# williamleif/GraphSAGE

Measured on NVIDIA H100. Metric: seed_nodes_per_sec, higher is better.
Workload: dtype f32

## Files before the change

### graphsage_b200/csrc/gemm_tc.cu

```cuda
#include "tc_common.cuh"

namespace gs {

constexpr int TC_THREADS = 256;

struct TcPart {
  const float* A;
  int64_t lda;
  int32_t K;
  int32_t N;
  int32_t kblocks;
  int32_t ntiles;
  int64_t img_off;
  const float* B;
  int64_t ldb;
};

struct TcParams {
  TcPart p[2];
  int32_t n_parts;
  int32_t combine;
  int64_t M;
  const float* bias;
  int32_t act;
  float* out;
  int64_t ldo;
  int32_t tiles_n0;
  gs_gemm_row_ids rid[2];
};

template <int MODE>
__global__ void __launch_bounds__(256) pack_b_kernel(TcParams prm, unsigned char* __restrict__ ws) {
  constexpr int BK = MODE == 2 ? 64 : 32;
  constexpr int EPC = MODE == 2 ? 8 : 4;
  constexpr int NIMG = MODE == 0 ? 2 : 1;
  int unit = blockIdx.x;
  int pi = 0;
  if (prm.n_parts == 2 && unit >= prm.p[0].ntiles * prm.p[0].kblocks) {
    unit -= prm.p[0].ntiles * prm.p[0].kblocks;
    pi = 1;
  }
  const TcPart& P = prm.p[pi];
  const int nt = unit / P.kblocks, kb = unit % P.kblocks;
  unsigned char* img = ws + P.img_off + ((int64_t)(nt * P.kblocks + kb) * NIMG) * TC_TILE_BYTES;
  for (int q = threadIdx.x; q < 128 * 8; q += blockDim.x) {
    const int c = q >> 7, n = q & 127;
    const int gn = nt * TC_BN + n;
    const int k0 = kb * BK + c * EPC;
    float w[EPC];
#pragma unroll
    for (int e = 0; e < EPC; ++e) w[e] = (gn < P.N && k0 + e < P.K) ? P.B[(int64_t)(k0 + e) * P.ldb + gn] : 0.f;
    const uint32_t off = sw128_off(n, c);
    if constexpr (MODE == 2) {
      __nv_bfloat162 h[4];
#pragma unroll
      for (int e = 0; e < 4; ++e) h[e] = __floats2bfloat162_rn(w[2 * e], w[2 * e + 1]);
      *reinterpret_cast<uint4*>(img + off) = *reinterpret_cast<uint4*>(h);
    } else {
      uint4 hi;
      hi.x = tf32_mask(w[0]); hi.y = tf32_mask(w[1]); hi.z = tf32_mask(w[2]); hi.w = tf32_mask(w[3]);
      *reinterpret_cast<uint4*>(img + off) = hi;
      if constexpr (MODE == 0) {
        uint4 lo;
        lo.x = tf32_mask(w[0] - __uint_as_float(hi.x)); lo.y = tf32_mask(w[1] - __uint_as_float(hi.y));
        lo.z = tf32_mask(w[2] - __uint_as_float(hi.z)); lo.w = tf32_mask(w[3] - __uint_as_float(hi.w));
        *reinterpret_cast<uint4*>(img + TC_TILE_BYTES + off) = lo;
      }
    }
  }
}

template <int MODE>
struct TcCfg {
  static constexpr int BK = MODE == 2 ? 64 : 32;
  static constexpr int NIMG = MODE == 0 ? 2 : 1;
  static constexpr int IMG_BYTES = NIMG * TC_TILE_BYTES;
  static constexpr int STAGES = MODE == 0 ? 3 : 4;
  static constexpr int STAGE_BYTES = 2 * IMG_BYTES;
  static constexpr int SMEM_BYTES = STAGES * STAGE_BYTES + 1024;
  static constexpr int CPT = 4;
};

template <int MODE>
__device__ __forceinline__ void load_a_chunk(const TcPart& P, int64_t arow, int gcol, bool vec, float (&v)[8]) {
  constexpr int EPC = MODE == 2 ? 8 : 4;
#pragma unroll
  for (int e = 0; e < 8; ++e) v[e] = 0.f;
  if (arow < 0) return;
  const float* src = P.A + arow * P.lda + gcol;
  if (vec && gcol + EPC <= P.K) {
    float4 a = ldg_nc_f4(reinterpret_cast<const float4*>(src));
    v[0] = a.x; v[1] = a.y; v[2] = a.z; v[3] = a.w;
    if constexpr (EPC == 8) {
      float4 b = ldg_nc_f4(reinterpret_cast<const float4*>(src) + 1);
      v[4] = b.x; v[5] = b.y; v[6] = b.z; v[7] = b.w;
    }
  } else {
#pragma unroll
    for (int e = 0; e < EPC; ++e)
      if (gcol + e < P.K) v[e] = __ldg(src + e);
  }
}

template <int MODE>
__device__ __forceinline__ void store_a_chunk(unsigned char* tile, int row, int c, const float (&v)[8]) {
  const uint32_t off = sw128_off(row, c);
  if constexpr (MODE == 2) {
    __nv_bfloat162 h[4];
#pragma unroll
    for (int e = 0; e < 4; ++e) h[e] = __floats2bfloat162_rn(v[2 * e], v[2 * e + 1]);
    *reinterpret_cast<uint4*>(tile + off) = *reinterpret_cast<uint4*>(h);
  } else {
    uint4 hi;
    hi.x = tf32_mask(v[0]); hi.y = tf32_mask(v[1]); hi.z = tf32_mask(v[2]); hi.w = tf32_mask(v[3]);
    *reinterpret_cast<uint4*>(tile + off) = hi;
    if constexpr (MODE == 0) {
      uint4 lo;
      lo.x = tf32_mask(v[0] - __uint_as_float(hi.x)); lo.y = tf32_mask(v[1] - __uint_as_float(hi.y));
      lo.z = tf32_mask(v[2] - __uint_as_float(hi.z)); lo.w = tf32_mask(v[3] - __uint_as_float(hi.w));
      *reinterpret_cast<uint4*>(tile + TC_TILE_BYTES + off) = lo;
    }
  }
}

template <int MODE>
__global__ void __launch_bounds__(TC_THREADS, 1) sage_gemm_tc_kernel(const __grid_constant__ TcParams prm,
                                                                     const unsigned char* __restrict__ ws) {
  using C = TcCfg<MODE>;
  extern __shared__ unsigned char smem_raw[];
  __shared__ __align__(8) uint64_t full[C::STAGES];

  unsigned char* smem = reinterpret_cast<unsigned char*>((reinterpret_cast<uintptr_t>(smem_raw) + 1023) & ~(uintptr_t)1023);
  const int tid = threadIdx.x, wg = tid >> 7, lane = tid & 31, wq = (tid >> 5) & 3;

  const int64_t m0 = (int64_t)blockIdx.x * TC_BM;
  int part_lo = 0, part_hi = prm.n_parts, ntile = blockIdx.y, col_off = 0;
  if (prm.combine == GS_COMBINE_CONCAT && prm.n_parts == 2) {
    if ((int)blockIdx.y < prm.tiles_n0) part_hi = 1;
    else { part_lo = 1; ntile = blockIdx.y - prm.tiles_n0; col_off = prm.p[0].N; }
  }
  const int N = prm.p[part_lo].N;
  int total_it = 0;
  for (int pi = part_lo; pi < part_hi; ++pi) total_it += prm.p[pi].kblocks;
  auto locate = [&](int it, int& pi, int& kb) {
    pi = part_lo; kb = it;
    while (kb >= prm.p[pi].kblocks) { kb -= prm.p[pi].kblocks; ++pi; }
  };

  if (tid == 0) {
    for (int s = 0; s < C::STAGES; ++s) mbar_init(&full[s], 1);
    fence_mbar_init();
  }
  __syncthreads();

  auto post = [&](int it) {
    if (tid != 0 || it >= total_it) return;
    int pi, kb;
    locate(it, pi, kb);
    const TcPart& P = prm.p[pi];
    const int s = it % C::STAGES;
    unsigned char* st = smem + (size_t)s * C::STAGE_BYTES;
    mbar_expect_tx(&full[s], C::IMG_BYTES);
    bulk_g2s(st + C::IMG_BYTES, ws + P.img_off + ((int64_t)ntile * P.kblocks + kb) * C::IMG_BYTES, C::IMG_BYTES, &full[s]);
  };
  int64_t arow_lo[C::CPT], arow_hi[C::CPT];
#pragma unroll
  for (int i = 0; i < C::CPT; ++i) {
    const int64_t r = m0 + ((tid + TC_THREADS * i) >> 3);
    arow_lo[i] = gemm_a_row(prm.rid[part_lo], prm.M, r);
    arow_hi[i] = part_hi - part_lo == 2 ? gemm_a_row(prm.rid[part_lo + 1], prm.M, r) : -1;
  }
  float cur[C::CPT][8];
  auto fetch = [&](int it) {
    int pi, kb;
    locate(it, pi, kb);
    const TcPart& P = prm.p[pi];
    const bool vec = ((P.lda & 3) == 0) && ((reinterpret_cast<uintptr_t>(P.A) & 15u) == 0);
#pragma unroll
    for (int i = 0; i < C::CPT; ++i) {
      const int q = tid + TC_THREADS * i;
      load_a_chunk<MODE>(P, pi == part_lo ? arow_lo[i] : arow_hi[i], kb * C::BK + (q & 7) * (MODE == 2 ? 8 : 4), vec, cur[i]);
    }
  };

  for (int j = 0; j < C::STAGES - 1; ++j) post(j);
  fetch(0);

  float acc[64];
#pragma unroll
  for (int i = 0; i < 64; ++i) acc[i] = 0.f;
  for (int it = 0; it < total_it; ++it) {
    const int s = it % C::STAGES;
    unsigned char* st = smem + (size_t)s * C::STAGE_BYTES;
#pragma unroll
    for (int i = 0; i < C::CPT; ++i) {
      const int q = tid + TC_THREADS * i;
      store_a_chunk<MODE>(st, q >> 3, q & 7, cur[i]);
    }
    fence_proxy_async();
    __syncthreads();
    post(it + C::STAGES - 1);
    if (it + 1 < total_it) fetch(it + 1);
    mbar_wait(&full[s], (uint32_t)(it / C::STAGES) & 1u);
    const uint32_t a_base = smem_u32(st) + (uint32_t)(wg * 64 * 128), b_base = smem_u32(st + C::IMG_BYTES);
    const uint64_t a_hi = make_smem_desc(a_base), b_hi = make_smem_desc(b_base);
    const uint64_t a_lo = make_smem_desc(a_base + TC_TILE_BYTES), b_lo = make_smem_desc(b_base + TC_TILE_BYTES);
    acc_fence(acc);
    wgmma_fence();
#pragma unroll
    for (int k = 0; k < 4; ++k) {
      const uint64_t koff = (uint64_t)((k * 32) >> 4);
      wgmma_m64n128<MODE == 2>(acc, a_hi + koff, b_hi + koff, (it > 0 || k > 0) ? 1u : 0u);
      if constexpr (MODE == 0) {
        wgmma_m64n128<false>(acc, a_hi + koff, b_lo + koff, 1u);
        wgmma_m64n128<false>(acc, a_lo + koff, b_hi + koff, 1u);
      }
    }
    wgmma_commit();
    wgmma_wait<0>();
    acc_fence(acc);
  }

#pragma unroll
  for (int h = 0; h < 2; ++h) {
    const int64_t grow = m0 + wg * 64 + wq * 16 + (lane >> 2) + 8 * h;
    if (grow >= prm.M) continue;
    float* dst_row = prm.out + grow * prm.ldo + col_off;
#pragma unroll
    for (int j = 0; j < 16; ++j) {
      const int gn = ntile * TC_BN + 8 * j + 2 * (lane & 3);
      float v[2];
#pragma unroll
      for (int e = 0; e < 2; ++e) {
        v[e] = acc[4 * j + 2 * h + e];
        if (prm.bias && gn + e < N) v[e] += prm.bias[col_off + gn + e];
        if (prm.act == GS_ACT_RELU) v[e] = fmaxf(v[e], 0.f);
      }
      float* dst = dst_row + gn;
      if (gn + 2 <= N && (reinterpret_cast<uintptr_t>(dst) & 7u) == 0) {
        *reinterpret_cast<float2*>(dst) = make_float2(v[0], v[1]);
      } else {
        if (gn < N) dst[0] = v[0];
        if (gn + 1 < N) dst[1] = v[1];
      }
    }
  }
}

static int mode_of(int32_t math) { return math == GS_MATH_TF32X3 ? 0 : math == GS_MATH_TF32 ? 1 : 2; }

static void fill_parts(TcParams& prm, int64_t M, const gs_gemm_part* parts, int32_t n_parts, int mode) {
  const int BK = mode == 2 ? 64 : 32;
  const int nimg = mode == 0 ? 2 : 1;
  memset(&prm, 0, sizeof(prm));
  prm.n_parts = n_parts;
  prm.M = M;
  int64_t off = 0;
  for (int i = 0; i < n_parts; ++i) {
    TcPart& P = prm.p[i];
    P.A = parts[i].A; P.lda = parts[i].lda; P.K = parts[i].K; P.N = parts[i].N;
    P.B = parts[i].B; P.ldb = parts[i].ldb;
    P.kblocks = (P.K + BK - 1) / BK;
    P.ntiles = (P.N + TC_BN - 1) / TC_BN;
    P.img_off = off;
    off += (int64_t)P.kblocks * P.ntiles * nimg * TC_TILE_BYTES;
  }
  prm.tiles_n0 = prm.p[0].ntiles;
}

int64_t sage_gemm_tc_workspace(int64_t M, const gs_gemm_part* parts, int32_t n_parts, int32_t math) {
  TcParams prm;
  fill_parts(prm, M, parts, n_parts, mode_of(math));
  const TcPart& L = prm.p[n_parts - 1];
  const int nimg = mode_of(math) == 0 ? 2 : 1;
  return L.img_off + (int64_t)L.kblocks * L.ntiles * nimg * TC_TILE_BYTES;
}

template <int MODE>
static int32_t launch_pack(const TcParams& prm, unsigned char* ws, cudaStream_t st) {
  int units = prm.p[0].ntiles * prm.p[0].kblocks + (prm.n_parts == 2 ? prm.p[1].ntiles * prm.p[1].kblocks : 0);
  pack_b_kernel<MODE><<<units, 256, 0, st>>>(prm, ws);
  return launch_check("pack_b_kernel");
}

template <int MODE>
static int32_t launch_tc(const TcParams& prm, const unsigned char* ws, cudaStream_t st) {
  using C = TcCfg<MODE>;
  const int32_t rc_attr = ensure_dyn_smem((const void*)sage_gemm_tc_kernel<MODE>, C::SMEM_BYTES);
  if (rc_attr != GS_OK) return rc_attr;
  int tiles_n = prm.p[0].ntiles;
  if (prm.combine == GS_COMBINE_CONCAT && prm.n_parts == 2) tiles_n += prm.p[1].ntiles;
  dim3 grid((unsigned)((prm.M + TC_BM - 1) / TC_BM), (unsigned)tiles_n);
  sage_gemm_tc_kernel<MODE><<<grid, TC_THREADS, C::SMEM_BYTES, st>>>(prm, ws);
  return launch_check("sage_gemm_tc_kernel");
}

int32_t sage_gemm_tc_pack(const gs_gemm_part* parts, int32_t n_parts, int32_t math, void* workspace, cudaStream_t st) {
  GS_REQUIRE(workspace != nullptr && (reinterpret_cast<uintptr_t>(workspace) & 127u) == 0,
             "gs_sage_gemm_pack: workspace must be non-NULL and 128-byte aligned");
  const int mode = mode_of(math);
  TcParams prm;
  fill_parts(prm, 0, parts, n_parts, mode);
  unsigned char* ws = (unsigned char*)workspace;
  if (mode == 0) return launch_pack<0>(prm, ws, st);
  if (mode == 1) return launch_pack<1>(prm, ws, st);
  return launch_pack<2>(prm, ws, st);
}

int32_t sage_gemm_tc(int64_t M, const gs_gemm_part* parts, const gs_gemm_row_ids* row_ids, int32_t n_parts, int32_t combine,
                     const float* bias, int32_t act, int32_t math, float* out, int64_t ldo, const void* workspace,
                     cudaStream_t st) {
  GS_REQUIRE(workspace != nullptr, "gs_sage_gemm: tensor-core math modes need the workspace (gs_sage_gemm_workspace_bytes)");
  GS_REQUIRE((reinterpret_cast<uintptr_t>(workspace) & 127u) == 0, "gs_sage_gemm: workspace must be 128-byte aligned");
  const int mode = mode_of(math);
  TcParams prm;
  fill_parts(prm, M, parts, n_parts, mode);
  for (int i = 0; row_ids && i < n_parts; ++i) prm.rid[i] = row_ids[i];
  prm.combine = combine;
  prm.bias = bias;
  prm.act = act;
  prm.out = out;
  prm.ldo = ldo;
  const unsigned char* ws = (const unsigned char*)workspace;
  if (mode == 0) return launch_tc<0>(prm, ws, st);
  if (mode == 1) return launch_tc<1>(prm, ws, st);
  return launch_tc<2>(prm, ws, st);
}

}
```

### graphsage_b200/csrc/layer_small.cu

```cuda
#include "common.cuh"

namespace gs {

constexpr int LS_ROWS = 4;
constexpr int LS_THREADS = 512;

struct LsParams {
  const float* src;
  int64_t n_src_rows, pitch;
  int32_t F;
  gs_segment seg;
  int32_t include_self;
  gs_gemm_part p[2];
  int32_t n_parts, combine;
  const float* bias;
  int32_t act, l2norm;
  float* out;
  int64_t ldo;
  uint64_t* counter_dev;
  uint64_t counter_inc;
  int32_t vec;
};

__device__ __forceinline__ int64_t ls_clamp(int64_t id, int64_t n) { return (id < 0 || id >= n) ? n - 1 : id; }

__global__ void __launch_bounds__(LS_THREADS) sage_layer_small_kernel(const __grid_constant__ LsParams prm) {
  extern __shared__ float sm[];
  const int F = prm.F;
  float* xs = sm;
  float* xm = sm + LS_ROWS * F;
  const gs_segment& sg = prm.seg;
  const int k = sg.k;
  const int64_t row0 = (int64_t)blockIdx.x * LS_ROWS;
  if (prm.vec) {
    const int f4 = F >> 2;
    for (int p = threadIdx.x; p < f4 * LS_ROWS; p += LS_THREADS) {
      const int r = p / f4, c4 = p - r * f4;
      const int64_t i = row0 + r;
      float4 acc = make_float4(0.f, 0.f, 0.f, 0.f), sv = acc;
      if (i < sg.n) {
        const int64_t srow = ls_clamp(sg.self_ids ? (int64_t)sg.self_ids[i] : sg.self_row0 + i, prm.n_src_rows);
        sv = ldg_nc_f4(reinterpret_cast<const float4*>(prm.src + srow * prm.pitch) + c4);
        for (int j0 = 0; j0 < k; j0 += 5) {
          float4 v[5];
#pragma unroll
          for (int u = 0; u < 5; ++u) {
            v[u] = make_float4(0.f, 0.f, 0.f, 0.f);
            if (j0 + u < k) {
              const int64_t nr = ls_clamp(sg.neigh_ids ? (int64_t)sg.neigh_ids[i * k + j0 + u] : sg.neigh_row0 + i * k + j0 + u,
                                          prm.n_src_rows);
              v[u] = ldg_nc_f4(reinterpret_cast<const float4*>(prm.src + nr * prm.pitch) + c4);
            }
          }
#pragma unroll
          for (int u = 0; u < 5; ++u) { acc.x += v[u].x; acc.y += v[u].y; acc.z += v[u].z; acc.w += v[u].w; }
        }
        const float div = (float)(k + (prm.include_self ? 1 : 0));
        if (prm.include_self) { acc.x += sv.x; acc.y += sv.y; acc.z += sv.z; acc.w += sv.w; }
        acc.x /= div; acc.y /= div; acc.z /= div; acc.w /= div;
      }
      reinterpret_cast<float4*>(xs + r * F)[c4] = sv;
      reinterpret_cast<float4*>(xm + r * F)[c4] = acc;
    }
  } else
  for (int c = threadIdx.x; c < F; c += LS_THREADS) {
    float acc[LS_ROWS], sv[LS_ROWS];
#pragma unroll
    for (int r = 0; r < LS_ROWS; ++r) {
      acc[r] = 0.f;
      const int64_t i = row0 + r;
      sv[r] = 0.f;
      if (i < sg.n) {
        const int64_t srow = ls_clamp(sg.self_ids ? (int64_t)sg.self_ids[i] : sg.self_row0 + i, prm.n_src_rows);
        sv[r] = prm.src[srow * prm.pitch + c];
      }
    }
    for (int j0 = 0; j0 < k; j0 += 5) {
      float v[LS_ROWS][5];
#pragma unroll
      for (int r = 0; r < LS_ROWS; ++r) {
        const int64_t i = row0 + r;
#pragma unroll
        for (int u = 0; u < 5; ++u) {
          v[r][u] = 0.f;
          if (i < sg.n && j0 + u < k) {
            const int64_t nr = ls_clamp(sg.neigh_ids ? (int64_t)sg.neigh_ids[i * k + j0 + u] : sg.neigh_row0 + i * k + j0 + u,
                                        prm.n_src_rows);
            v[r][u] = prm.src[nr * prm.pitch + c];
          }
        }
      }
#pragma unroll
      for (int r = 0; r < LS_ROWS; ++r)
#pragma unroll
        for (int u = 0; u < 5; ++u) acc[r] += v[r][u];
    }
#pragma unroll
    for (int r = 0; r < LS_ROWS; ++r) {
      float a = acc[r];
      if (prm.include_self) a += sv[r];
      a /= (float)(k + (prm.include_self ? 1 : 0));
      xs[r * F + c] = sv[r];
      xm[r * F + c] = (row0 + r < sg.n) ? a : 0.f;
    }
  }
  __syncthreads();
  const int N0 = prm.p[0].N;
  const int ntot = (prm.n_parts == 2 && prm.combine == GS_COMBINE_CONCAT) ? N0 + prm.p[1].N : N0;
  const int ncolp = (ntot + 31) & ~31;
  const int ncgp = prm.vec ? ((((ntot + 3) >> 2) + 31) & ~31) : 0;
  const int nslices = prm.vec ? (ncgp <= LS_THREADS ? LS_THREADS / ncgp : 1) : (ncolp <= LS_THREADS ? LS_THREADS / ncolp : 1);
  float* part = xm + LS_ROWS * F;
  float* red = part + nslices * LS_ROWS * ncolp;
  if (prm.vec) {
    const int ncg = ntot >> 2;
    const int sl = threadIdx.x / ncgp;
    const int cg0 = threadIdx.x - sl * ncgp;
    for (int cg = cg0; cg < ncg && sl < nslices; cg += (nslices == 1 ? LS_THREADS : ncgp)) {
      const int col = cg * 4;
      float4 acc[LS_ROWS];
#pragma unroll
      for (int r = 0; r < LS_ROWS; ++r) acc[r] = make_float4(0.f, 0.f, 0.f, 0.f);
      for (int pi = 0; pi < prm.n_parts; ++pi) {
        int c = col;
        if (prm.n_parts == 2 && prm.combine == GS_COMBINE_CONCAT) {
          if ((pi == 0) != (col < N0)) continue;
          if (pi == 1) c = col - N0;
        }
        const gs_gemm_part& P = prm.p[pi];
        const float* x = (prm.n_parts == 1 || pi == 1) ? xm : xs;
        const float* w = P.B + c;
        const int kchunk = (((P.K + nslices - 1) / nslices) + 3) & ~3;
        const int kbeg = sl * kchunk, kend = min(P.K, kbeg + kchunk);
        float4 wn[4];
        if (kbeg < kend) {
#pragma unroll
          for (int u = 0; u < 4; ++u) wn[u] = __ldg(reinterpret_cast<const float4*>(w + (int64_t)(kbeg + u) * P.ldb));
        }
        for (int kk = kbeg; kk < kend; kk += 4) {
          float4 wv[4];
#pragma unroll
          for (int u = 0; u < 4; ++u) wv[u] = wn[u];
          if (kk + 4 < kend) {
#pragma unroll
            for (int u = 0; u < 4; ++u) wn[u] = __ldg(reinterpret_cast<const float4*>(w + (int64_t)(kk + 4 + u) * P.ldb));
          }
#pragma unroll
          for (int r = 0; r < LS_ROWS; ++r) {
            const float4 xv = *reinterpret_cast<const float4*>(x + r * F + kk);
            acc[r].x = fmaf(xv.x, wv[0].x, acc[r].x); acc[r].y = fmaf(xv.x, wv[0].y, acc[r].y);
            acc[r].z = fmaf(xv.x, wv[0].z, acc[r].z); acc[r].w = fmaf(xv.x, wv[0].w, acc[r].w);
            acc[r].x = fmaf(xv.y, wv[1].x, acc[r].x); acc[r].y = fmaf(xv.y, wv[1].y, acc[r].y);
            acc[r].z = fmaf(xv.y, wv[1].z, acc[r].z); acc[r].w = fmaf(xv.y, wv[1].w, acc[r].w);
            acc[r].x = fmaf(xv.z, wv[2].x, acc[r].x); acc[r].y = fmaf(xv.z, wv[2].y, acc[r].y);
            acc[r].z = fmaf(xv.z, wv[2].z, acc[r].z); acc[r].w = fmaf(xv.z, wv[2].w, acc[r].w);
            acc[r].x = fmaf(xv.w, wv[3].x, acc[r].x); acc[r].y = fmaf(xv.w, wv[3].y, acc[r].y);
            acc[r].z = fmaf(xv.w, wv[3].z, acc[r].z); acc[r].w = fmaf(xv.w, wv[3].w, acc[r].w);
          }
        }
      }
#pragma unroll
      for (int r = 0; r < LS_ROWS; ++r) *reinterpret_cast<float4*>(part + (sl * LS_ROWS + r) * ncolp + col) = acc[r];
      if (nslices > 1) break;
    }
  }
  const int slice = prm.vec ? nslices : (nslices == 1 ? 0 : threadIdx.x / ncolp);
  const int col_step = nslices == 1 ? LS_THREADS : ncolp;
  for (int col = (nslices == 1 ? threadIdx.x : threadIdx.x % ncolp); col < ntot && slice < nslices; col += col_step) {
    float acc[LS_ROWS];
#pragma unroll
    for (int r = 0; r < LS_ROWS; ++r) acc[r] = 0.f;
    for (int pi = 0; pi < prm.n_parts; ++pi) {
      int c = col;
      if (prm.n_parts == 2 && prm.combine == GS_COMBINE_CONCAT) {
        if ((pi == 0) != (col < N0)) continue;
        if (pi == 1) c = col - N0;
      }
      const gs_gemm_part& P = prm.p[pi];
      const float* x = (prm.n_parts == 1 || pi == 1) ? xm : xs;
      const float* w = P.B + c;
      const int kchunk = (((P.K + nslices - 1) / nslices) + 7) & ~7;
      const int kbeg = slice * kchunk, kend = min(P.K, kbeg + kchunk);
      int kk = kbeg;
      for (; kk + 8 <= kend; kk += 8) {
        float wv[8];
#pragma unroll
        for (int u = 0; u < 8; ++u) wv[u] = __ldg(w + (int64_t)(kk + u) * P.ldb);
#pragma unroll
        for (int u = 0; u < 8; ++u)
#pragma unroll
          for (int r = 0; r < LS_ROWS; ++r) acc[r] = fmaf(x[r * F + kk + u], wv[u], acc[r]);
      }
      for (; kk < kend; ++kk) {
        const float wv = __ldg(w + (int64_t)kk * P.ldb);
#pragma unroll
        for (int r = 0; r < LS_ROWS; ++r) acc[r] = fmaf(x[r * F + kk], wv, acc[r]);
      }
    }
#pragma unroll
    for (int r = 0; r < LS_ROWS; ++r) part[(slice * LS_ROWS + r) * ncolp + col] = acc[r];
    if (nslices > 1) break;
  }
  __syncthreads();
  float ss[LS_ROWS];
#pragma unroll
  for (int r = 0; r < LS_ROWS; ++r) ss[r] = 0.f;
  for (int col = threadIdx.x; col < ntot; col += LS_THREADS) {
#pragma unroll
    for (int r = 0; r < LS_ROWS; ++r) {
      float v = 0.f;
      for (int s2 = 0; s2 < nslices; ++s2) v += part[(s2 * LS_ROWS + r) * ncolp + col];
      if (prm.bias) v += prm.bias[col];
      if (prm.act == GS_ACT_RELU) v = fmaxf(v, 0.f);
      ss[r] += v * v;
      part[r * ncolp + col] = v;
    }
  }
  float inv[LS_ROWS];
#pragma unroll
  for (int r = 0; r < LS_ROWS; ++r) inv[r] = 1.f;
  if (prm.l2norm) {
#pragma unroll
    for (int r = 0; r < LS_ROWS; ++r) {
      float t = ss[r];
#pragma unroll
      for (int o = 16; o > 0; o >>= 1) t += __shfl_xor_sync(0xffffffffu, t, o);
      if ((threadIdx.x & 31) == 0) red[r * 16 + (threadIdx.x >> 5)] = t;
    }
    __syncthreads();
#pragma unroll
    for (int r = 0; r < LS_ROWS; ++r) {
      float tot = 0.f;
#pragma unroll
      for (int w = 0; w < LS_THREADS / 32; ++w) tot += red[r * 16 + w];
      inv[r] = 1.0f / sqrtf(fmaxf(tot, 1e-12f));
    }
  }
  for (int col = threadIdx.x; col < ntot; col += LS_THREADS) {
#pragma unroll
    for (int r = 0; r < LS_ROWS; ++r)
      if (row0 + r < sg.n) prm.out[(sg.out_row0 + row0 + r) * prm.ldo + col] = part[r * ncolp + col] * inv[r];
  }
  if (prm.counter_dev != nullptr && blockIdx.x == 0 && threadIdx.x == 0) *prm.counter_dev += prm.counter_inc;
}

}

extern "C" int32_t gs_sage_layer_small(const float* src, int64_t n_src_rows, int32_t F, int64_t pitch,
                                       const gs_segment* segment_host, int32_t include_self,
                                       const gs_gemm_part* parts_host, int32_t n_parts, int32_t combine, const float* bias,
                                       int32_t act, int32_t l2_normalize, float* out, int64_t ldo, uint64_t* counter_dev,
                                       uint64_t counter_inc, void* stream) {
  GS_REQUIRE(src && segment_host && parts_host && out, "gs_sage_layer_small: NULL pointer");
  GS_REQUIRE(n_parts == 1 || n_parts == 2, "gs_sage_layer_small: n_parts=%d", n_parts);
  GS_REQUIRE(F >= 1 && F <= 2048 && pitch >= F && n_src_rows > 0, "gs_sage_layer_small: F=%d (max 2048) / pitch", F);
  GS_REQUIRE(segment_host->k >= 1 && segment_host->n >= 0, "gs_sage_layer_small: bad segment");
  GS_REQUIRE(combine == GS_COMBINE_ADD || combine == GS_COMBINE_CONCAT, "gs_sage_layer_small: combine=%d", combine);
  GS_REQUIRE(act == GS_ACT_NONE || act == GS_ACT_RELU, "gs_sage_layer_small: act=%d", act);
  gs::LsParams prm;
  memset(&prm, 0, sizeof(prm));
  int ntot = 0;
  for (int i = 0; i < n_parts; ++i) {
    GS_REQUIRE(parts_host[i].B && parts_host[i].K == F && parts_host[i].N >= 1 && parts_host[i].ldb >= parts_host[i].N,
               "gs_sage_layer_small: part %d must have K == F (%d) and a valid B", i, F);
    prm.p[i] = parts_host[i];
  }
  if (n_parts == 2 && combine == GS_COMBINE_ADD)
    GS_REQUIRE(parts_host[0].N == parts_host[1].N, "gs_sage_layer_small: ADD needs equal N");
  ntot = parts_host[0].N + ((n_parts == 2 && combine == GS_COMBINE_CONCAT) ? parts_host[1].N : 0);
  GS_REQUIRE(ntot <= 1024 && ldo >= ntot, "gs_sage_layer_small: output width %d (max 1024) / ldo", ntot);
  if (segment_host->n == 0) return GS_OK;
  prm.src = src; prm.n_src_rows = n_src_rows; prm.pitch = pitch; prm.F = F;
  prm.seg = *segment_host; prm.include_self = include_self;
  prm.n_parts = n_parts; prm.combine = combine; prm.bias = bias; prm.act = act; prm.l2norm = l2_normalize;
  prm.out = out; prm.ldo = ldo; prm.counter_dev = counter_dev; prm.counter_inc = counter_inc;
  bool vec = (F % 4 == 0) && (pitch % 4 == 0) && ((reinterpret_cast<uintptr_t>(src) & 15u) == 0) && (ntot % 4 == 0) &&
             (parts_host[0].N % 4 == 0);
  for (int i = 0; i < n_parts; ++i)
    vec = vec && (parts_host[i].ldb % 4 == 0) && ((reinterpret_cast<uintptr_t>(parts_host[i].B) & 15u) == 0);
  prm.vec = vec ? 1 : 0;
  const int ncolp = (ntot + 31) & ~31;
  const int ncgp = (((ntot + 3) / 4) + 31) & ~31;
  const int nslices = vec ? (ncgp <= gs::LS_THREADS ? gs::LS_THREADS / ncgp : 1)
                          : (ncolp <= gs::LS_THREADS ? gs::LS_THREADS / ncolp : 1);
  const size_t smem = (size_t)(2 * gs::LS_ROWS * F + nslices * gs::LS_ROWS * ncolp + gs::LS_ROWS * 16) * sizeof(float);
  GS_REQUIRE(smem <= 200 * 1024, "gs_sage_layer_small: needs %zu bytes of shared memory", smem);
  {
    const int32_t rc_attr = gs::ensure_dyn_smem((const void*)gs::sage_layer_small_kernel, 200 * 1024);
    if (rc_attr != GS_OK) return rc_attr;
  }
  unsigned blocks = (unsigned)((segment_host->n + gs::LS_ROWS - 1) / gs::LS_ROWS);
  gs::sage_layer_small_kernel<<<blocks, gs::LS_THREADS, smem, (cudaStream_t)stream>>>(prm);
  return gs::launch_check("sage_layer_small_kernel");
}
```

### graphsage_b200/csrc/sampler.cu

```cuda
#include "common.cuh"

namespace gs {

constexpr int kMaxDegSmem = 1024;

__global__ void __launch_bounds__(256) sample_padded_kernel(const int32_t* __restrict__ adj, int64_t n_rows,
                                                            int32_t max_deg, const int32_t* __restrict__ ids,
                                                            int64_t n, int32_t k,
                                                            const int32_t* __restrict__ col_perm, uint64_t seed,
                                                            uint64_t counter, const uint64_t* __restrict__ counter_dev,
                                                            int32_t* __restrict__ out) {
  __shared__ int16_t perm[kMaxDegSmem];
  __shared__ int32_t pi[kMaxDegSmem];
  if (col_perm != nullptr) {
    for (int j = threadIdx.x; j < k; j += blockDim.x) pi[j] = col_perm[j];
  } else {
    for (int j = threadIdx.x; j < max_deg; j += blockDim.x) perm[j] = (int16_t)j;
    __syncthreads();
    if (threadIdx.x == 0) {
      uint64_t ctr = counter + (counter_dev ? *counter_dev : 0ull);
      u32x4 r{0, 0, 0, 0};
      for (int i = 0; i < k; ++i) {
        if ((i & 3) == 0) {
          u32x4 c{(uint32_t)ctr, (uint32_t)(ctr >> 32), 0u, kStreamPadded + (uint32_t)(i >> 2)};
          r = philox4x32_10(c, (uint32_t)seed, (uint32_t)(seed >> 32));
        }
        int j = i + (int)mulhi32(pick(r, i & 3), (uint32_t)(max_deg - i));
        int16_t t = perm[i];
        perm[i] = perm[j];
        perm[j] = t;
        pi[i] = perm[i];
      }
    }
  }
  __syncthreads();
  const int64_t total = n * (int64_t)k;
  for (int64_t e = (int64_t)blockIdx.x * blockDim.x + threadIdx.x; e < total; e += (int64_t)gridDim.x * blockDim.x) {
    int64_t i = e / k;
    int j = (int)(e - i * k);
    int64_t id = ids[i];
    if (id < 0 || id >= n_rows) id = n_rows - 1;
    out[e] = adj[id * max_deg + pi[j]];
  }
}

struct KhopParams {
  int32_t* out[GS_MAX_HOPS];
  int32_t fanout[GS_MAX_HOPS];
  int64_t count[GS_MAX_HOPS];
  int32_t n_hops;
};

__global__ void __launch_bounds__(512) sample_padded_khop_kernel(const int32_t* __restrict__ adj, int64_t n_rows,
                                                                 int32_t max_deg, const int32_t* __restrict__ seeds,
                                                                 const __grid_constant__ KhopParams kp, uint64_t seed,
                                                                 uint64_t counter,
                                                                 const uint64_t* __restrict__ counter_dev) {
  __shared__ int16_t perm[GS_MAX_HOPS][kMaxDegSmem];
  __shared__ int32_t pi[GS_MAX_HOPS][64];
  const int warp = threadIdx.x >> 5, lane = threadIdx.x & 31;
  if (warp < kp.n_hops) {
    for (int j = lane; j < max_deg; j += 32) perm[warp][j] = (int16_t)j;
    __syncwarp();
    const uint64_t ctr = counter + (counter_dev ? *counter_dev : 0ull) + (uint64_t)warp;
    const int k = kp.fanout[warp];
    for (int blk = lane; blk * 4 < k; blk += 32) {
      u32x4 c{(uint32_t)ctr, (uint32_t)(ctr >> 32), 0u, kStreamPadded + (uint32_t)blk};
      u32x4 r = philox4x32_10(c, (uint32_t)seed, (uint32_t)(seed >> 32));
      pi[warp][blk * 4 + 0] = (int32_t)r.x;
      if (blk * 4 + 1 < 64) pi[warp][blk * 4 + 1] = (int32_t)r.y;
      if (blk * 4 + 2 < 64) pi[warp][blk * 4 + 2] = (int32_t)r.z;
      if (blk * 4 + 3 < 64) pi[warp][blk * 4 + 3] = (int32_t)r.w;
    }
    __syncwarp();
    if (lane == 0) {
      for (int i = 0; i < k; ++i) {
        int j = i + (int)mulhi32((uint32_t)pi[warp][i], (uint32_t)(max_deg - i));
        int16_t t = perm[warp][i];
        perm[warp][i] = perm[warp][j];
        perm[warp][j] = t;
        pi[warp][i] = perm[warp][i];
      }
    }
  }
  __syncthreads();
  int64_t total = 0;
  for (int t = 0; t < kp.n_hops; ++t) total += kp.count[t];
  for (int64_t e = (int64_t)blockIdx.x * blockDim.x + threadIdx.x; e < total; e += (int64_t)gridDim.x * blockDim.x) {
    int hop = 0;
    int64_t local = e;
    while (local >= kp.count[hop]) { local -= kp.count[hop]; ++hop; }
    int64_t sup = 1;
    for (int t = 0; t <= hop; ++t) sup *= kp.fanout[t];
    int64_t id = seeds[local / sup];
    int64_t rem = local % sup;
    for (int t = 0; t <= hop; ++t) {
      sup /= kp.fanout[t];
      const int j = (int)(rem / sup);
      rem -= (int64_t)j * sup;
      if (id < 0 || id >= n_rows) id = n_rows - 1;
      id = adj[id * max_deg + pi[t][j]];
    }
    kp.out[hop][local] = (int32_t)id;
  }
}

__global__ void __launch_bounds__(256) sample_csr_kernel(const int64_t* __restrict__ indptr,
                                                         const int32_t* __restrict__ indices, int64_t n_nodes,
                                                         const int32_t* __restrict__ ids, int64_t n, int32_t k,
                                                         int32_t replace_if_short, uint64_t seed, uint64_t counter,
                                                         const uint64_t* __restrict__ counter_dev, int32_t pad_id,
                                                         int32_t* __restrict__ out) {
  const int lane = threadIdx.x & 31;
  const int64_t warp = ((int64_t)blockIdx.x * blockDim.x + threadIdx.x) >> 5;
  const int64_t nwarps = ((int64_t)gridDim.x * blockDim.x) >> 5;
  const uint64_t ctr = counter + (counter_dev ? *counter_dev : 0ull);
  for (int64_t t = warp; t < n; t += nwarps) {
    int64_t id = ids[t];
    int64_t start = 0, deg = 0;
    if (id >= 0 && id < n_nodes) {
      start = indptr[id];
      deg = indptr[id + 1] - start;
    }
    int32_t res = pad_id;
    uint32_t r = 0;
    if (lane < k && deg > 0) r = philox_draw(seed, ctr, (uint32_t)t, kStreamCsr, lane);
    if (deg >= k) {
      int64_t mine = -1;
      for (int j = 0; j < k; ++j) {
        uint32_t rj = __shfl_sync(0xffffffffu, r, j);
        int64_t m = deg - k + j;
        int64_t tpos = (int64_t)mulhi32(rj, (uint32_t)(m + 1));
        unsigned dup = __ballot_sync(0xffffffffu, lane < j && mine == tpos);
        if (lane == j) mine = dup ? m : tpos;
      }
      if (lane < k) res = indices[start + mine];
    } else if (deg > 0) {
      if (replace_if_short) {
        if (lane < k) res = indices[start + (int64_t)mulhi32(r, (uint32_t)deg)];
      } else {
        if (lane < deg) res = indices[start + lane];
      }
    }
    if (lane < k) out[t * k + lane] = res;
  }
}

__global__ void __launch_bounds__(128) sample_unigram_kernel(const double* __restrict__ cdf, int64_t n, int32_t num,
                                                             uint64_t seed, uint64_t counter,
                                                             const uint64_t* __restrict__ counter_dev,
                                                             int32_t* __restrict__ out) {
  const int j = blockIdx.x * blockDim.x + threadIdx.x;
  if (j >= num) return;
  const uint64_t ctr = counter + (counter_dev ? *counter_dev : 0ull);
  const uint32_t r = philox_draw(seed, ctr, 0u, kStreamUnigram, j);
  const double u = ((double)r + 0.5) * (1.0 / 4294967296.0) * cdf[n - 1];
  int64_t lo = 0, hi = n - 1;
  while (lo < hi) {
    const int64_t mid = (lo + hi) >> 1;
    if (cdf[mid] > u) hi = mid; else lo = mid + 1;
  }
  out[j] = (int32_t)lo;
}

__device__ __forceinline__ int32_t unigram_lookup(const double* __restrict__ cdf, int64_t n, uint32_t r) {
  const double u = ((double)r + 0.5) * (1.0 / 4294967296.0) * cdf[n - 1];
  int64_t lo = 0, hi = n - 1;
  while (lo < hi) {
    const int64_t mid = (lo + hi) >> 1;
    if (cdf[mid] > u) hi = mid; else lo = mid + 1;
  }
  return (int32_t)lo;
}

__global__ void __launch_bounds__(32) sample_unigram_unique_kernel(const double* __restrict__ cdf, int64_t n, int32_t num,
                                                                   int64_t max_draws, uint64_t seed, uint64_t counter,
                                                                   const uint64_t* __restrict__ counter_dev,
                                                                   int32_t* __restrict__ out, int32_t* __restrict__ status) {
  __shared__ int32_t held[GS_MAX_UNIQUE_SAMPLED];
  const unsigned FULL = 0xffffffffu;
  const int lane = threadIdx.x;
  const unsigned lower = (1u << lane) - 1u;
  const uint64_t ctr = counter + (counter_dev ? *counter_dev : 0ull);
  int count = 0;
  int64_t j0 = 0;
  for (; count < num && j0 < max_draws; j0 += 32) {
    const int64_t j = j0 + lane;
    const bool live = j < max_draws;
      const int32_t id = live ? unigram_lookup(cdf, n, philox_draw(seed, ctr, 0u, kStreamUnigramUnique, (int)j)) : -1 - lane;
    bool fresh = live;
    for (int q = 0; q < count; ++q) fresh &= held[q] != id;
    const unsigned same = __match_any_sync(FULL, id);
    fresh &= (same & lower) == 0u;
    const unsigned acc = __ballot_sync(FULL, fresh);
    const int pos = count + __popc(acc & lower);
    if (fresh && pos < num) {
      held[pos] = id;
      out[pos] = id;
    }
    count = min(num, count + __popc(acc));
    __syncwarp();
  }
  for (int p = count + lane; p < num; p += 32) out[p] = -1;
  if (lane == 0 && status != nullptr && count < num) *status = 1;
}

__global__ void __launch_bounds__(256) build_padded_adj_kernel(const int64_t* __restrict__ indptr,
                                                               const int32_t* __restrict__ indices, int64_t n_nodes,
                                                               int32_t max_deg, const uint8_t* __restrict__ skip,
                                                               uint64_t seed, uint64_t counter, int32_t* __restrict__ adj,
                                                               float* __restrict__ deg_out) {
  __shared__ int32_t sel[8][kMaxDegSmem];
  const int lane = threadIdx.x & 31, w = threadIdx.x >> 5;
  const int64_t warp = (int64_t)blockIdx.x * 8 + w;
  const int64_t nwarps = (int64_t)gridDim.x * 8;
  for (int64_t u = warp; u <= n_nodes; u += nwarps) {
    int32_t* row = adj + u * max_deg;
    int64_t start = 0, deg = 0;
    if (u < n_nodes && !(skip && skip[u])) {
      start = indptr[u];
      deg = indptr[u + 1] - start;
    }
    if (u < n_nodes && deg_out && lane == 0) deg_out[u] = (float)deg;
    if (deg == 0) {
      for (int j = lane; j < max_deg; j += 32) row[j] = (int32_t)n_nodes;
    } else if (deg == max_deg) {
      for (int j = lane; j < max_deg; j += 32) row[j] = indices[start + j];
    } else if (deg < max_deg) {
      for (int j = lane; j < max_deg; j += 32) {
        const uint32_t r = philox_draw(seed, counter, (uint32_t)u, kStreamBuild, j);
        row[j] = indices[start + (int64_t)mulhi32(r, (uint32_t)deg)];
      }
    } else {
      for (int j = 0; j < max_deg; ++j) {
        const int64_t m = deg - max_deg + j;
        const uint32_t r = philox_draw(seed, counter, (uint32_t)u, kStreamBuild, j);
        const int32_t t = (int32_t)mulhi32(r, (uint32_t)(m + 1));
        bool dup = false;
        for (int q = lane; q < j; q += 32) dup |= (sel[w][q] == t);
        dup = __any_sync(0xffffffffu, dup);
        if (lane == 0) sel[w][j] = dup ? (int32_t)m : t;
        __syncwarp();
      }
      for (int j = lane; j < max_deg; j += 32) row[j] = indices[start + sel[w][j]];
      __syncwarp();
    }
  }
}

}

extern "C" {

int32_t gs_sample_padded(const int32_t* adj, int64_t n_rows, int32_t max_deg, const int32_t* ids, int64_t n, int32_t k,
                         const int32_t* col_perm, uint64_t seed, uint64_t counter, const uint64_t* counter_dev,
                         int32_t* out, void* stream) {
  GS_REQUIRE(n >= 0 && k >= 0, "gs_sample_padded: negative size (n=%lld, k=%d)", (long long)n, k);
  if (n == 0 || k == 0) return GS_OK;
  GS_REQUIRE(adj && ids && out, "gs_sample_padded: NULL pointer");
  GS_REQUIRE(n_rows > 0 && max_deg > 0 && max_deg <= gs::kMaxDegSmem, "gs_sample_padded: need 0 < max_deg <= %d (got %d)",
             gs::kMaxDegSmem, max_deg);
  GS_REQUIRE(k <= max_deg, "gs_sample_padded: num_samples %d > max_degree %d", k, max_deg);
  int64_t total = n * (int64_t)k;
  int64_t blocks = (total + 255) / 256;
  int64_t cap = (int64_t)gs::sm_count() * 8;
  if (blocks > cap) blocks = cap;
  gs::sample_padded_kernel<<<(unsigned)blocks, 256, 0, (cudaStream_t)stream>>>(adj, n_rows, max_deg, ids, n, k, col_perm,
                                                                               seed, counter, counter_dev, out);
  return gs::launch_check("sample_padded_kernel");
}

int32_t gs_sample_padded_khop(const int32_t* adj, int64_t n_rows, int32_t max_deg, const int32_t* seeds, int64_t n_seeds,
                              const int32_t* fanout_host, int32_t n_hops, uint64_t seed, uint64_t counter,
                              const uint64_t* counter_dev, int32_t* const* out_host, void* stream) {
  GS_REQUIRE(n_hops >= 1 && n_hops <= GS_MAX_HOPS, "gs_sample_padded_khop: n_hops=%d (max %d)", n_hops, GS_MAX_HOPS);
  GS_REQUIRE(fanout_host && out_host, "gs_sample_padded_khop: NULL host array");
  GS_REQUIRE(n_seeds >= 0, "gs_sample_padded_khop: n_seeds < 0");
  if (n_seeds == 0) return GS_OK;
  GS_REQUIRE(adj && seeds, "gs_sample_padded_khop: NULL pointer");
  GS_REQUIRE(n_rows > 0 && max_deg > 0 && max_deg <= gs::kMaxDegSmem, "gs_sample_padded_khop: need 0 < max_deg <= %d",
             gs::kMaxDegSmem);
  gs::KhopParams kp;
  memset(&kp, 0, sizeof(kp));
  kp.n_hops = n_hops;
  int64_t cnt = n_seeds, total = 0;
  for (int t = 0; t < n_hops; ++t) {
    GS_REQUIRE(fanout_host[t] >= 1 && fanout_host[t] <= max_deg && fanout_host[t] <= 64,
               "gs_sample_padded_khop: fanout[%d]=%d (need 1..min(64, max_degree))", t, fanout_host[t]);
    GS_REQUIRE(out_host[t] != nullptr, "gs_sample_padded_khop: out[%d] is NULL", t);
    cnt *= fanout_host[t];
    kp.fanout[t] = fanout_host[t];
    kp.count[t] = cnt;
    kp.out[t] = out_host[t];
    total += cnt;
  }
  int64_t blocks = (total + 511) / 512;
  int64_t cap = (int64_t)gs::sm_count() * 2;
  if (blocks > cap) blocks = cap;
  gs::sample_padded_khop_kernel<<<(unsigned)blocks, 512, 0, (cudaStream_t)stream>>>(adj, n_rows, max_deg, seeds, kp, seed,
                                                                                    counter, counter_dev);
  return gs::launch_check("sample_padded_khop_kernel");
}

int32_t gs_build_padded_adj(const int64_t* indptr, const int32_t* indices, int64_t n_nodes, int32_t max_deg,
                            const uint8_t* skip, uint64_t seed, uint64_t counter, int32_t* adj, float* deg, void* stream) {
  GS_REQUIRE(indptr && indices && adj && n_nodes >= 0, "gs_build_padded_adj: NULL pointer / bad size");
  GS_REQUIRE(max_deg >= 1 && max_deg <= gs::kMaxDegSmem, "gs_build_padded_adj: need 1 <= max_deg <= %d", gs::kMaxDegSmem);
  int64_t blocks = (n_nodes + 1 + 7) / 8;
  int64_t cap = (int64_t)gs::sm_count() * 4;
  if (blocks > cap) blocks = cap;
  gs::build_padded_adj_kernel<<<(unsigned)blocks, 256, 0, (cudaStream_t)stream>>>(indptr, indices, n_nodes, max_deg, skip,
                                                                                   seed, counter, adj, deg);
  return gs::launch_check("build_padded_adj_kernel");
}

int32_t gs_sample_unigram(const double* cdf, int64_t n, int32_t num_sampled, uint64_t seed, uint64_t counter,
                          const uint64_t* counter_dev, int32_t* out, void* stream) {
  GS_REQUIRE(num_sampled >= 0 && n >= 1, "gs_sample_unigram: bad sizes");
  if (num_sampled == 0) return GS_OK;
  GS_REQUIRE(cdf && out, "gs_sample_unigram: NULL pointer");
  gs::sample_unigram_kernel<<<(num_sampled + 127) / 128, 128, 0, (cudaStream_t)stream>>>(cdf, n, num_sampled, seed, counter,
                                                                                       counter_dev, out);
  return gs::launch_check("sample_unigram_kernel");
}

int32_t gs_sample_unigram_unique(const double* cdf, int64_t n, int32_t num_sampled, uint64_t seed, uint64_t counter,
                                 const uint64_t* counter_dev, int32_t* out, int32_t* status, void* stream) {
  GS_REQUIRE(n >= 1 && n < 0x7fffffffLL, "gs_sample_unigram_unique: need 1 <= n < 2^31 - 1 (got %lld)", (long long)n);
  GS_REQUIRE(num_sampled >= 0 && num_sampled <= GS_MAX_UNIQUE_SAMPLED && num_sampled <= n,
             "gs_sample_unigram_unique: num_sampled=%d must be in [0, min(%d, n=%lld)]", num_sampled, GS_MAX_UNIQUE_SAMPLED,
             (long long)n);
  if (num_sampled == 0) return GS_OK;
  GS_REQUIRE(cdf && out, "gs_sample_unigram_unique: NULL pointer");
  gs::sample_unigram_unique_kernel<<<1, 32, 0, (cudaStream_t)stream>>>(cdf, n, num_sampled, GS_UNIQUE_DRAW_BUDGET, seed,
                                                                      counter, counter_dev, out, status);
  return gs::launch_check("sample_unigram_unique_kernel");
}

int32_t gs_sample_csr(const int64_t* indptr, const int32_t* indices, int64_t n_nodes, const int32_t* ids, int64_t n,
                      int32_t k, int32_t replace_if_short, uint64_t seed, uint64_t counter, const uint64_t* counter_dev,
                      int32_t pad_id, int32_t* out, void* stream) {
  GS_REQUIRE(n >= 0 && k >= 0, "gs_sample_csr: negative size");
  if (n == 0 || k == 0) return GS_OK;
  GS_REQUIRE(indptr && indices && ids && out, "gs_sample_csr: NULL pointer");
  if (k > 32) {
    gs::set_error("gs_sample_csr: k=%d > 32 not supported (one lane per draw)", k);
    return GS_ERR_UNSUPPORTED;
  }
  int64_t blocks = (n + 7) / 8;
  int64_t cap = (int64_t)gs::sm_count() * 8;
  if (blocks > cap) blocks = cap;
  gs::sample_csr_kernel<<<(unsigned)blocks, 256, 0, (cudaStream_t)stream>>>(indptr, indices, n_nodes, ids, n, k,
                                                                            replace_if_short, seed, counter, counter_dev,
                                                                            pad_id, out);
  return gs::launch_check("sample_csr_kernel");
}

}
```

Before: 3.559 million.

## Overlap wgmma with next stage, halve small-layer and sampler block sizes

The tensor-core GEMM now keeps one wgmma group in flight (wait<1>) and prefetches one fewer stage ahead so the buffer being overwritten is no longer being read. The small-layer kernel drops to 256 threads, each handling two logical lanes, with a register cap and a reshaped shared-memory layout that lets the partial-sum region overlap the input rows. The k-hop sampler uses 256-thread blocks with a larger block cap. Together these target latency hiding and occupancy, at the cost of a shallower TMA prefetch, possible register spills, and extra syncs.

```diff
diff --git a/graphsage_b200/csrc/gemm_tc.cu b/graphsage_b200/csrc/gemm_tc.cu
--- a/graphsage_b200/csrc/gemm_tc.cu
+++ b/graphsage_b200/csrc/gemm_tc.cu
@@ -183,7 +183,7 @@
     }
   };
 
-  for (int j = 0; j < C::STAGES - 1; ++j) post(j);
+  for (int j = 0; j < C::STAGES - 2; ++j) post(j);
   fetch(0);
 
   float acc[64];
@@ -199,7 +199,7 @@
     }
     fence_proxy_async();
     __syncthreads();
-    post(it + C::STAGES - 1);
+    post(it + C::STAGES - 2);
     if (it + 1 < total_it) fetch(it + 1);
     mbar_wait(&full[s], (uint32_t)(it / C::STAGES) & 1u);
     const uint32_t a_base = smem_u32(st) + (uint32_t)(wg * 64 * 128), b_base = smem_u32(st + C::IMG_BYTES);
@@ -217,9 +217,11 @@
       }
     }
     wgmma_commit();
-    wgmma_wait<0>();
+    wgmma_wait<1>();
     acc_fence(acc);
   }
+  wgmma_wait<0>();
+  acc_fence(acc);
 
 #pragma unroll
   for (int h = 0; h < 2; ++h) {
diff --git a/graphsage_b200/csrc/layer_small.cu b/graphsage_b200/csrc/layer_small.cu
--- a/graphsage_b200/csrc/layer_small.cu
+++ b/graphsage_b200/csrc/layer_small.cu
@@ -3,7 +3,15 @@
 namespace gs {
 
 constexpr int LS_ROWS = 4;
-constexpr int LS_THREADS = 512;
+constexpr int LS_THREADS = 256;
+constexpr int LS_LANES = 2 * LS_THREADS;
+
+__host__ __device__ __forceinline__ int ls_part_offset(int F, int ncgp, int ncolp, int vec) {
+  const int x = 2 * LS_ROWS * F;
+  if (!vec || ncgp > LS_THREADS) return x;
+  const int o = x - (LS_THREADS / ncgp) * LS_ROWS * ncolp;
+  return o > 0 ? o : 0;
+}
 
 struct LsParams {
   const float* src;
@@ -24,7 +32,7 @@
 
 __device__ __forceinline__ int64_t ls_clamp(int64_t id, int64_t n) { return (id < 0 || id >= n) ? n - 1 : id; }
 
-__global__ void __launch_bounds__(LS_THREADS) sage_layer_small_kernel(const __grid_constant__ LsParams prm) {
+__global__ void __maxnreg__(72) sage_layer_small_kernel(const __grid_constant__ LsParams prm) {
   extern __shared__ float sm[];
   const int F = prm.F;
   float* xs = sm;
@@ -109,14 +117,19 @@
   const int ntot = (prm.n_parts == 2 && prm.combine == GS_COMBINE_CONCAT) ? N0 + prm.p[1].N : N0;
   const int ncolp = (ntot + 31) & ~31;
   const int ncgp = prm.vec ? ((((ntot + 3) >> 2) + 31) & ~31) : 0;
-  const int nslices = prm.vec ? (ncgp <= LS_THREADS ? LS_THREADS / ncgp : 1) : (ncolp <= LS_THREADS ? LS_THREADS / ncolp : 1);
-  float* part = xm + LS_ROWS * F;
+  const int nslices = prm.vec ? (ncgp <= LS_LANES ? LS_LANES / ncgp : 1) : (ncolp <= LS_LANES ? LS_LANES / ncolp : 1);
+  float* part = sm + ls_part_offset(F, ncgp, ncolp, prm.vec);
   float* red = part + nslices * LS_ROWS * ncolp;
   if (prm.vec) {
     const int ncg = ntot >> 2;
-    const int sl = threadIdx.x / ncgp;
-    const int cg0 = threadIdx.x - sl * ncgp;
-    for (int cg = cg0; cg < ncg && sl < nslices; cg += (nslices == 1 ? LS_THREADS : ncgp)) {
+    float4 held[LS_ROWS];
+    int held_col = -1, held_sl = 0;
+#pragma unroll
+    for (int h = 1; h >= 0; --h) {
+    const int lane_id = threadIdx.x + h * LS_THREADS;
+    const int sl = lane_id / ncgp;
+    const int cg0 = lane_id - sl * ncgp;
+    for (int cg = cg0; cg < ncg && sl < nslices; cg += (nslices == 1 ? LS_LANES : ncgp)) {
       const int col = cg * 4;
       float4 acc[LS_ROWS];
 #pragma unroll
@@ -159,14 +172,29 @@
           }
         }
       }
-#pragma unroll
-      for (int r = 0; r < LS_ROWS; ++r) *reinterpret_cast<float4*>(part + (sl * LS_ROWS + r) * ncolp + col) = acc[r];
+      if (h == 0 && nslices > 1) {
+#pragma unroll
+        for (int r = 0; r < LS_ROWS; ++r) held[r] = acc[r];
+        held_col = col;
+        held_sl = sl;
+      } else {
+#pragma unroll
+        for (int r = 0; r < LS_ROWS; ++r) *reinterpret_cast<float4*>(part + (sl * LS_ROWS + r) * ncolp + col) = acc[r];
+      }
       if (nslices > 1) break;
     }
-  }
-  const int slice = prm.vec ? nslices : (nslices == 1 ? 0 : threadIdx.x / ncolp);
-  const int col_step = nslices == 1 ? LS_THREADS : ncolp;
-  for (int col = (nslices == 1 ? threadIdx.x : threadIdx.x % ncolp); col < ntot && slice < nslices; col += col_step) {
+    }
+    __syncthreads();
+    if (held_col >= 0) {
+#pragma unroll
+      for (int r = 0; r < LS_ROWS; ++r) *reinterpret_cast<float4*>(part + (held_sl * LS_ROWS + r) * ncolp + held_col) = held[r];
+    }
+  }
+  for (int h = 0; h < 2 && !prm.vec; ++h) {
+  const int lane_id = threadIdx.x + h * LS_THREADS;
+  const int slice = nslices == 1 ? 0 : lane_id / ncolp;
+  const int col_step = nslices == 1 ? LS_LANES : ncolp;
+  for (int col = (nslices == 1 ? lane_id : lane_id % ncolp); col < ntot && slice < nslices; col += col_step) {
     float acc[LS_ROWS];
 #pragma unroll
     for (int r = 0; r < LS_ROWS; ++r) acc[r] = 0.f;
@@ -201,19 +229,23 @@
     for (int r = 0; r < LS_ROWS; ++r) part[(slice * LS_ROWS + r) * ncolp + col] = acc[r];
     if (nslices > 1) break;
   }
+  }
   __syncthreads();
-  float ss[LS_ROWS];
-#pragma unroll
-  for (int r = 0; r < LS_ROWS; ++r) ss[r] = 0.f;
-  for (int col = threadIdx.x; col < ntot; col += LS_THREADS) {
-#pragma unroll
-    for (int r = 0; r < LS_ROWS; ++r) {
-      float v = 0.f;
-      for (int s2 = 0; s2 < nslices; ++s2) v += part[(s2 * LS_ROWS + r) * ncolp + col];
-      if (prm.bias) v += prm.bias[col];
-      if (prm.act == GS_ACT_RELU) v = fmaxf(v, 0.f);
-      ss[r] += v * v;
-      part[r * ncolp + col] = v;
+  float ss[2][LS_ROWS];
+#pragma unroll
+  for (int h = 0; h < 2; ++h) {
+#pragma unroll
+    for (int r = 0; r < LS_ROWS; ++r) ss[h][r] = 0.f;
+    for (int col = threadIdx.x + h * LS_THREADS; col < ntot; col += LS_LANES) {
+#pragma unroll
+      for (int r = 0; r < LS_ROWS; ++r) {
+        float v = 0.f;
+        for (int s2 = 0; s2 < nslices; ++s2) v += part[(s2 * LS_ROWS + r) * ncolp + col];
+        if (prm.bias) v += prm.bias[col];
+        if (prm.act == GS_ACT_RELU) v = fmaxf(v, 0.f);
+        ss[h][r] += v * v;
+        part[r * ncolp + col] = v;
+      }
     }
   }
   float inv[LS_ROWS];
@@ -221,18 +253,21 @@
   for (int r = 0; r < LS_ROWS; ++r) inv[r] = 1.f;
   if (prm.l2norm) {
 #pragma unroll
-    for (int r = 0; r < LS_ROWS; ++r) {
-      float t = ss[r];
-#pragma unroll
-      for (int o = 16; o > 0; o >>= 1) t += __shfl_xor_sync(0xffffffffu, t, o);
-      if ((threadIdx.x & 31) == 0) red[r * 16 + (threadIdx.x >> 5)] = t;
+    for (int h = 0; h < 2; ++h) {
+#pragma unroll
+      for (int r = 0; r < LS_ROWS; ++r) {
+        float t = ss[h][r];
+#pragma unroll
+        for (int o = 16; o > 0; o >>= 1) t += __shfl_xor_sync(0xffffffffu, t, o);
+        if ((threadIdx.x & 31) == 0) red[r * 16 + ((threadIdx.x + h * LS_THREADS) >> 5)] = t;
+      }
     }
     __syncthreads();
 #pragma unroll
     for (int r = 0; r < LS_ROWS; ++r) {
       float tot = 0.f;
 #pragma unroll
-      for (int w = 0; w < LS_THREADS / 32; ++w) tot += red[r * 16 + w];
+      for (int w = 0; w < LS_LANES / 32; ++w) tot += red[r * 16 + w];
       inv[r] = 1.0f / sqrtf(fmaxf(tot, 1e-12f));
     }
   }
@@ -281,9 +316,10 @@
   prm.vec = vec ? 1 : 0;
   const int ncolp = (ntot + 31) & ~31;
   const int ncgp = (((ntot + 3) / 4) + 31) & ~31;
-  const int nslices = vec ? (ncgp <= gs::LS_THREADS ? gs::LS_THREADS / ncgp : 1)
-                          : (ncolp <= gs::LS_THREADS ? gs::LS_THREADS / ncolp : 1);
-  const size_t smem = (size_t)(2 * gs::LS_ROWS * F + nslices * gs::LS_ROWS * ncolp + gs::LS_ROWS * 16) * sizeof(float);
+  const int nslices = vec ? (ncgp <= gs::LS_LANES ? gs::LS_LANES / ncgp : 1)
+                          : (ncolp <= gs::LS_LANES ? gs::LS_LANES / ncolp : 1);
+  const size_t smem = (size_t)(gs::ls_part_offset(F, ncgp, ncolp, vec ? 1 : 0) + nslices * gs::LS_ROWS * ncolp +
+                               gs::LS_ROWS * 16) * sizeof(float);
   GS_REQUIRE(smem <= 200 * 1024, "gs_sage_layer_small: needs %zu bytes of shared memory", smem);
   {
     const int32_t rc_attr = gs::ensure_dyn_smem((const void*)gs::sage_layer_small_kernel, 200 * 1024);
diff --git a/graphsage_b200/csrc/sampler.cu b/graphsage_b200/csrc/sampler.cu
--- a/graphsage_b200/csrc/sampler.cu
+++ b/graphsage_b200/csrc/sampler.cu
@@ -44,6 +44,7 @@
   }
 }
 
+constexpr int kKhopThreads = 256;
 struct KhopParams {
   int32_t* out[GS_MAX_HOPS];
   int32_t fanout[GS_MAX_HOPS];
@@ -51,7 +52,7 @@
   int32_t n_hops;
 };
 
-__global__ void __launch_bounds__(512) sample_padded_khop_kernel(const int32_t* __restrict__ adj, int64_t n_rows,
+__global__ void __launch_bounds__(kKhopThreads) sample_padded_khop_kernel(const int32_t* __restrict__ adj, int64_t n_rows,
                                                                  int32_t max_deg, const int32_t* __restrict__ seeds,
                                                                  const __grid_constant__ KhopParams kp, uint64_t seed,
                                                                  uint64_t counter,
@@ -294,11 +295,12 @@
     kp.out[t] = out_host[t];
     total += cnt;
   }
-  int64_t blocks = (total + 511) / 512;
-  int64_t cap = (int64_t)gs::sm_count() * 2;
+  int64_t blocks = (total + gs::kKhopThreads - 1) / gs::kKhopThreads;
+  int64_t cap = (int64_t)gs::sm_count() * 4;
   if (blocks > cap) blocks = cap;
-  gs::sample_padded_khop_kernel<<<(unsigned)blocks, 512, 0, (cudaStream_t)stream>>>(adj, n_rows, max_deg, seeds, kp, seed,
-                                                                                    counter, counter_dev);
+  gs::sample_padded_khop_kernel<<<(unsigned)blocks, gs::kKhopThreads, 0, (cudaStream_t)stream>>>(adj, n_rows, max_deg, seeds,
+                                                                                                 kp, seed, counter,
+                                                                                                 counter_dev);
   return gs::launch_check("sample_padded_khop_kernel");
 }
 
```

Measured after the change: 3.656 million, median of 6. +2.7%, better.
